# var-nan/SGUFP_Solver

Measured on AMD Instinct MI355X. Metric: B&B-node relaxations/sec + achieved HBM GB/s, 1k-arc 256-scenario synthetic, higher is better.
Workload: dtype f64

## Files before the change

include/sgufp_hip.h:

```cpp
#ifndef SGUFP_HIP_H
#define SGUFP_HIP_H

#include <stdint.h>

#ifdef __cplusplus
extern "C" {
#endif

typedef struct sgufp_ctx sgufp_ctx;

#define SGUFP_OK 0
#define SGUFP_ERR_ARG (-1)
#define SGUFP_ERR_NETWORK (-2)
#define SGUFP_ERR_HIP (-3)
#define SGUFP_ERR_CAPACITY (-4)
#define SGUFP_ERR_STATE (-5)
#define SGUFP_ERR_KEY (-6)

#define SGUFP_SUCCESS 0
#define SGUFP_PRUNED_BY_FEASIBILITY_CUT 1
#define SGUFP_PRUNED_BY_OPTIMALITY_CUT 2
#define SGUFP_NEEDS_SUBPROBLEM 3
#define SGUFP_PRUNED_BY_BOUND 4
#define SGUFP_NODE_ERR_RECORD 16
// ... 33 lines not shown
int sgufp_batch_upload(sgufp_ctx *ctx, int n, const uint16_t *global_layer, const double *lb, const double *ub,
                       const int64_t *states_off, const int16_t *states, const int64_t *sol_off,
                       const int16_t *sol);
int sgufp_batch_relax(sgufp_ctx *ctx, double optimal_lb);
int sgufp_batch_sync(sgufp_ctx *ctx);
int sgufp_batch_results(sgufp_ctx *ctx, int32_t *status, uint8_t *exact, double *lb, double *ub,
                        int32_t *n_children);
int sgufp_batch_children_size(sgufp_ctx *ctx, int64_t *n_children, int64_t *n_states, int64_t *n_sol);
int sgufp_batch_children(sgufp_ctx *ctx, int64_t *child_off, uint16_t *global_layer, double *lb, double *ub,
                         int64_t *states_off, int16_t *states, int64_t *sol_off, int16_t *sol);
int sgufp_batch_paths(sgufp_ctx *ctx, int64_t *path_off, int16_t *paths);
int sgufp_batch_stats(sgufp_ctx *ctx, int64_t *dd_nodes, int64_t *dd_arcs, int32_t *dd_layers, int32_t *sweeps);
int sgufp_batch_refine(sgufp_ctx *ctx, int n, const int32_t *node_idx, const uint8_t *is_feasibility,
                       const int32_t *cut_index, double optimal_lb);

int sgufp_dd_build(sgufp_ctx *ctx);
int sgufp_dd_apply(sgufp_ctx *ctx, int node, int is_feasibility, double rhs, int64_t nnz, const uint64_t *keys,
                   const double *vals, double optimal, double *value);
int sgufp_dd_solution(sgufp_ctx *ctx, int node, int16_t *path, int32_t *len);
int sgufp_dd_cutset(sgufp_ctx *ctx, int node, double ub, int64_t *n_children);

int sgufp_batch_debug(sgufp_ctx *ctx, int64_t *ticks, int32_t *redo);
int sgufp_batch_phases(sgufp_ctx *ctx, int64_t *phase);
int sgufp_batch_refold_stats(sgufp_ctx *ctx, uint32_t *stats);

#define SGUFP_ROUTE_IN_ORDER 0
#define SGUFP_ROUTE_EXACT_PHASE 1
#define SGUFP_ROUTE_NX_PHASE 2
#define SGUFP_ROUTE_NX_FALLBACK 3
int sgufp_batch_routes(sgufp_ctx *ctx, int32_t *route);

int sgufp_subproblem(sgufp_ctx *ctx, int n, const int64_t *path_off, const int16_t *paths, int32_t *type,
                     double *rhs, double *rows, double *obj_mean);
int sgufp_subproblem_detail(sgufp_ctx *ctx, int32_t *status, double *objective, double *dual_objective);
int sgufp_subproblem_warm(sgufp_ctx *ctx, int n, const int64_t *path_off, const int16_t *paths, const int32_t *warm_src,
                          const int32_t *warm_dst, int32_t *type, double *rhs, double *rows, double *obj_mean);
int sgufp_subproblem_stats(sgufp_ctx *ctx, int32_t *augmentations, int32_t *passes);
int sgufp_subproblem_flows(sgufp_ctx *ctx, int n, const int64_t *path_off, const int16_t *paths, int32_t *status,
                           double *objective, double *flow_reward, int16_t *flows, double *mean_flow);
int sgufp_slot_keys(const sgufp_ctx *ctx, uint64_t *keys);
int sgufp_cuts_append_rows(sgufp_ctx *ctx, int is_feasibility, int n_cuts, const double *rhs, const double *rows);

typedef struct {
    int64_t popped;
    int64_t relaxed;
    int64_t pruned_bound;
// ... 74 lines not shown
```

sgufp_solver_amd/csrc/capi.cpp:

```cpp
#include <cstdio>

#include "ctx.hpp"
#include <algorithm>
#include <cstdlib>


namespace {

int64_t node_bound(const Network &net, int64_t *tail = nullptr) {
    const int L = net.L;
    auto set_size = [&](int sid) { return sid >= 0 ? (int)net.sets[sid].size() : 1; };
    int start = std::max(0, L - 5);
    std::vector<int64_t> h(kMaxStates + 2, 0);
    int c0 = set_size(net.layer_universe[start]);
    h[c0] = (L > 5) ? kRelaxedMaxWidth - 1 : 1;
    int64_t total = (int64_t)(kRelaxedMaxWidth - 1) * (start + 1);
    int64_t tail_nodes = 0;
    for (int l = start; l < L; l++) {
        if (net.layer_update[l] >= 0) {
            int64_t w = 0;
            for (auto x : h) w += x;
            std::fill(h.begin(), h.end(), 0);
            h[set_size(net.layer_update[l])] = w;
        }
// ... 97 lines not shown
    if (relax_lds_bytes(sc.Tcap, sc.Lcap, cb, sc.us) > 160 * 1024) { err = "too many layers for the LDS layer table"; return false; }
    sc.tmir_cap = cb > 1 ? (int)(sc.Ncap + sc.Acap) : 0;
    sc.tail_cap = (int)tail;
    sc.cb_max = cb;
    const size_t B = (size_t)max_batch;
    if (!alloc(sc.ntopo, B * sc.Ncap, "scratch") || !alloc(sc.nflag, B * sc.Ncap, "scratch") ||
        !alloc(sc.nmask, B * sc.Ncap, "scratch") || !alloc(sc.outcnt, B * sc.Ncap, "scratch") ||
        !alloc(sc.s2, B * sc.Ncap, "scratch") || !alloc(sc.tw, B * sc.Ncap, "scratch") ||
        !alloc(sc.atopo, B * sc.Acap, "scratch") || !alloc(sc.aflag, B * sc.Acap, "scratch") ||
        !alloc(sc.lay, B * sc.Tcap * 5, "scratch") || !alloc(sc.rslot, B * sc.Lcap, "scratch") ||
        !alloc(sc.meta, B * 8, "scratch") || !alloc(sc.ubv, B, "scratch") ||
        !alloc(sc.sm1, B * sc.Tcap, "scratch") || !alloc(sc.xm1, B * sc.Tcap, "scratch") ||
        !alloc(sc.v1, B * sc.Tcap, "scratch"))
        return false;
    if (cb > 1 && (!alloc(sc.s2b, B * sc.tail_cap * cb, "scratch") || !alloc(sc.sm, B * sc.Tcap * cb, "scratch") ||
                   !alloc(sc.xm, B * sc.Tcap * cb, "scratch") || !alloc(sc.tmir, B * (size_t)sc.tmir_cap, "scratch")))
        return false;
    if (const char *e = getenv("SGUFP_REFOLD_STATS"))
        if (atoi(e) != 0 && cb > 1 && !alloc(sc.rstat, B * kRefoldStats, "scratch")) return false;
    if (!alloc(out.status, B, "out") || !alloc(out.exact, B, "out") || !alloc(out.lb, B, "out") ||
        !alloc(out.ub, B, "out") || !alloc(out.nchild, B, "out") || !alloc(out.sol_need, B, "out") ||
        !alloc(out.dd_nodes, B, "out") || !alloc(out.dd_arcs, B, "out") || !alloc(out.dd_layers, B, "out") ||
        !alloc(out.sweeps, B, "out") || !alloc(out.path, B * sc.Lcap, "out") || !alloc(out.path_len, B, "out") ||
        !alloc(out.ticks, B, "out") || !alloc(out.redo, B, "out") || !alloc(out.phase, B * 8, "out"))
        return false;
    if (!alloc(d_gl, B, "batch") || !alloc(d_sollen, B, "batch") || !alloc(d_lb, B, "batch") ||
        !alloc(d_ub, B, "batch") || !alloc(d_mask, B, "batch") || !alloc(d_valid, B, "batch") ||
        !alloc(d_soloff, B, "batch") || !alloc(d_coff, B + 1, "batch") || !alloc(d_soff, B + 1, "batch") ||
        !alloc(d_rslots, B, "batch") || !alloc(d_rcuts, B, "batch") || !alloc(d_rfeas, B, "batch"))
        return false;
    sol_cap = B * (size_t)std::max(1, L);
    if (!alloc(d_sol, sol_cap, "batch")) return false;
    if (!alloc(d_bidx, B, "bnb") || !alloc(d_boff, B + 1, "bnb") || !alloc(d_bsol, B + 1, "bnb") ||
        !alloc(d_bpaths, B * (size_t)sc.Lcap, "bnb"))
        return false;
    if (!grow_rows(64)) return false;
    cur = staged();
    return sync();
}

bool sgufp_ctx::grow_rows(int need) {
    if (need <= row_cap) return true;
    int cap = std::max(need, row_cap * 2);
    const size_t stride = (size_t)net.n_slots + 1;
    const size_t tstride = (size_t)std::max(net.L, 1) * ustride;
    double *rows = nullptr, *rhs = nullptr, *coefT = nullptr;
    if (!alloc(rows, (size_t)cap * stride, "cut rows") || !alloc(rhs, (size_t)cap, "cut rhs") ||
// ... 1138 lines not shown
    std::vector<int32_t> rows(n);
    for (int k = 0; k < n; k++) {
        const auto &v = is_feasibility[k] ? ctx->f_rows : ctx->o_rows;
        if (node_idx[k] < 0 || node_idx[k] >= ctx->n || cut_index[k] < 0 || cut_index[k] >= (int)v.size())
            return SGUFP_ERR_ARG;
        rows[k] = v[cut_index[k]];
    }
    if (!ctx->upload(ctx->d_rslots, node_idx, n) || !ctx->upload(ctx->d_rcuts, rows.data(), n) ||
        !ctx->upload(ctx->d_rfeas, is_feasibility, n))
        return SGUFP_ERR_HIP;
    if (!ctx->hip_ok(launch_refine(ctx->nd, ctx->sc, ctx->batch(), ctx->pool(), ctx->out, ctx->d_rslots, ctx->d_rcuts,
                                   ctx->d_rfeas, n, optimal_lb, ctx->ex, ctx->stream),
                     "k_refine"))
        return SGUFP_ERR_HIP;
    return ctx->sync() ? SGUFP_OK : SGUFP_ERR_HIP;
}

int sgufp_batch_phases(sgufp_ctx *ctx, int64_t *phase) {
    if (!ctx || !ctx->relaxed || !phase) return ctx ? SGUFP_ERR_STATE : SGUFP_ERR_ARG;
    if (!relax_has_phases()) {
        std::fill(phase, phase + (size_t)ctx->n * 8, (int64_t)0);
        return SGUFP_OK;
    }
    std::vector<uint64_t> t((size_t)ctx->n * 8);
    if (!ctx->download(t.data(), ctx->out.phase, t.size()) || !ctx->sync()) return SGUFP_ERR_HIP;
    for (size_t k = 0; k < t.size(); k++) phase[k] = (int64_t)t[k];
    return SGUFP_OK;
}

int sgufp_batch_refold_stats(sgufp_ctx *ctx, uint32_t *stats) {
    if (!ctx || !stats) return SGUFP_ERR_ARG;
    if (!ctx->relaxed || !ctx->sc.rstat) return SGUFP_ERR_STATE;
    if (!ctx->download(stats, ctx->sc.rstat, (size_t)ctx->n * kRefoldStats) || !ctx->sync()) return SGUFP_ERR_HIP;
    return SGUFP_OK;
}

int sgufp_batch_debug(sgufp_ctx *ctx, int64_t *ticks, int32_t *redo) {
    if (!ctx || !ctx->relaxed) return ctx ? SGUFP_ERR_STATE : SGUFP_ERR_ARG;
    const int n = ctx->n;
    std::vector<uint64_t> t(n);
    std::vector<uint32_t> r(n);
    if (!ctx->download(t.data(), ctx->out.ticks, n) || !ctx->download(r.data(), ctx->out.redo, n) || !ctx->sync())
        return SGUFP_ERR_HIP;
    const bool stamped = relax_has_phases();
    for (int k = 0; k < n; k++) {
        if (ticks) ticks[k] = stamped ? (int64_t)t[k] : 0;
        if (redo) redo[k] = (int32_t)r[k];
    }
    return SGUFP_OK;
// ... 168 lines not shown
```

sgufp_solver_amd/csrc/dd_device.hpp:

```cpp
#pragma once

#include <cstdint>

#if defined(__HIP_DEVICE_COMPILE__) && !defined(SGUFP_HOST_ONLY)
#define SGUFP_GBL __attribute__((address_space(1)))
#else
#define SGUFP_GBL
#endif

namespace sgufp {

constexpr int kWave = 64;
constexpr int kMaxU = 32;
constexpr int kLdsWidth = 512;
constexpr int kBoundBlocks = 1024;

enum NodeStatus : int32_t {
    kSuccess = 0,
    kPrunedFeasibility = 1,
    kPrunedOptimality = 2,
    kNeedsSubproblem = 3,
    kPrunedBound = 4,
    kErrRecord = 16,
    kErrCapacity = 17,
// ... 95 lines not shown
    int ustride;
    const int32_t SGUFP_GBL *o_rank;
    int nscreen;
};

struct BatchOut {
    int32_t SGUFP_GBL *status;
    uint8_t SGUFP_GBL *exact;
    double SGUFP_GBL *lb;
    double SGUFP_GBL *ub;
    uint32_t SGUFP_GBL *nchild;
    uint32_t SGUFP_GBL *sol_need;
    uint32_t SGUFP_GBL *dd_nodes;
    uint32_t SGUFP_GBL *dd_arcs;
    uint32_t SGUFP_GBL *dd_layers;
    uint32_t SGUFP_GBL *sweeps;
    int16_t SGUFP_GBL *path;
    uint16_t SGUFP_GBL *path_len;
    uint64_t SGUFP_GBL *ticks;
    uint64_t SGUFP_GBL *phase;
    uint32_t SGUFP_GBL *redo;
};

struct ChildOut {
    const uint64_t SGUFP_GBL *child_off;
    const uint64_t SGUFP_GBL *sol_base;
    uint16_t SGUFP_GBL *gl;
    double SGUFP_GBL *lb;
    double SGUFP_GBL *ub;
    uint32_t SGUFP_GBL *mask;
    int64_t SGUFP_GBL *sol_off;
    uint16_t SGUFP_GBL *sol_len;
    int16_t SGUFP_GBL *sol;
};

constexpr int32_t kExactPending = 5;
#ifndef SGUFP_EXACT_MAXT
#define SGUFP_EXACT_MAXT 8
#endif
#ifndef SGUFP_EXACT_ENTRIES
#define SGUFP_EXACT_ENTRIES 40
#endif
#ifndef SGUFP_LEAVES_PER_WAVE
#define SGUFP_LEAVES_PER_WAVE 16
#endif
constexpr int kExactMaxT = SGUFP_EXACT_MAXT;
// ... 58 lines not shown
```

sgufp_solver_amd/csrc/dd_kernels.hip:

```cpp
#include <hip/hip_runtime.h>

#include <climits>
#include <cstdint>
#include <type_traits>

#include "dd_device.hpp"
#include "wave.hpp"

namespace sgufp {

#define DMIN (-__DBL_MAX__)
#define DMAX (__DBL_MAX__)

constexpr uint32_t kCollapseWidth = 120;


struct VP {
    double v;
    int p;
};
__device__ __forceinline__ VP vp_pick(VP a, VP b) {
    const bool take_b = (a.p == INT_MIN) | ((b.p != INT_MIN) & ((b.v > a.v) | (!(a.v > b.v) & (b.p > a.p))));
    VP r;
    r.v = take_b ? b.v : a.v;
// ... 695 lines not shown
    }
    for (uint32_t a = lane(); a < d.Amir; a += kWave) {
        uint32_t t = d.atopo[a];
        const bool al = (d.aflag[a] & kAlive) != 0;
        d.tmir[d.Nn + a] = (uint16_t)((al ? (t & kMirParent) : kNarrowMax) | (((t >> kRankShift) & 31u) << kMirRankShift) |
                                      (al ? kMirAlive : 0));
    }
    wave_mem_sync();
}

__device__ __forceinline__ void batch_coef_direct(const NetDev &net, const DD &d, BatchView &bv, const Pool &pool, int k,
                                         int nb) {
    const int us = pool.ustride, ls = d.g + k - 1;
    const size_t ltab = (size_t)net.L * us;
    for (int idx = lane(); idx < nb * us; idx += kWave) {
        int cc = idx / us, r = idx - cc * us;
        bv.coef[idx] = pool.coefT[(size_t)bv.ids[cc] * ltab + (size_t)ls * us + r];
    }
    wave_lds_sync();
}

template <int CB>
__device__ __forceinline__ void sweep_narrow(const NetDev &net, DD &d, BatchView &bv, const Pool &pool, int nb,
                                             double rv, int kS, int kend = INT_MAX) {
    constexpr int G = kWave / CB;
    constexpr int PC = kStageEntries / kWave, PT = kTopoEntries / kWave;
    const int c = lane() % CB, grp = lane() / CB;
    const bool cv = c < nb;
    const int us = pool.ustride;
    const int per_layer = nb * us;
    const size_t ltab = (size_t)net.L * us;
    if (lane() < CB && cv) {
        bv.vb[c] = rv;
        if (c == nb - 1) d.s2[0] = rv;
    }
    if (lane() < 2 * CB)
        bv.vb[(size_t)(lane() / CB) * kLdsBatchWidth * CB + kNarrowMax * CB + (lane() % CB)] = __builtin_nan("");
    if (d.ng == 0) return;
    double pf[PC] = {};
    uint32_t pt[PT] = {};
    uint32_t m_noff = 0, m_aoff = 0, m_pk = 0;
    uint64_t mmask = 0;
    int c_lo[PC];
    uint32_t c_off[PC];
    auto commit = [&](int slot, int gw) {
        LDS double *ring = bv.cring + (size_t)slot * kStageEntries;
        LDS uint16_t *tr = bv.tring + (size_t)slot * kTopoEntries;
// ... 31 lines not shown
        c_lo[jj] = lo | ((r == 0 && lo < 31 ? lo : 31) << 8);
        c_off[jj] = (uint32_t)(bv.ids[cc < nb ? cc : 0] * (int)ltab + r);
    }
    auto issue = [&](int k0g, int k1g, int lw0) {
        const uint32_t n0 = rl(m_noff, k0g - lw0), nN = rl(m_noff, k1g - lw0) - n0;
        const uint32_t a0 = rl(m_aoff, k0g - lw0), nA = rl(m_aoff, k1g - lw0) - a0;
#pragma unroll
        for (int jj = 0; jj < PC; jj++) {
            const int k = min(k0g + (c_lo[jj] & 255), k1g - 1);
            pf[jj] = pool.coefT[(size_t)c_off[jj] + (size_t)(uint32_t)((d.g + k - 1) * us)];
        }
#pragma unroll
        for (int jj = 0; jj < PT; jj++) {
            const uint32_t e = (uint32_t)(lane() + jj * kWave);
            const uint32_t idx = e < nN ? n0 + e : (e < nN + nA ? d.Nn + a0 + (e - nN) : 0u);
            pt[jj] = d.tmir[idx];
        }
    };

    auto fold_run = [&](auto Dc, int ka, int slot_, int k0_, int kw_, uint32_t gn0_) {
        constexpr int D = decltype(Dc)::value;
        const int kb = ka + D - 1;
        const LDS uint16_t *tr = bv.tring + (size_t)slot_ * kTopoEntries;
        const LDS double *ring_c = bv.cring + (size_t)slot_ * kStageEntries + c * us;
        const LDS double *pb = bv.vb + (size_t)((ka - 1) & 1) * kLdsBatchWidth * CB;
        LDS double *ob = bv.vb + (size_t)(kb & 1) * kLdsBatchWidth * CB;
        const int l0 = ka - k0_, lw = ka - kw_;
        uint32_t ebase[D], nofs[D];
        bool w1s[D], wrs[D];
        bool outs = false;
#pragma unroll
        for (int s = 0; s < D; s++) {
            nofs[s] = rl(m_noff, lw + s);
            ebase[s] = nofs[s] - gn0_;
            w1s[s] = (rl(m_pk, lw + s) >> 31) != 0;
            wrs[s] = ((rl(m_pk, lw + s) >> 30) & 1u) != 0;
            outs |= w1s[s] | wrs[s];
        }
        const uint32_t nlast = rl(m_pk, lw + D - 1) & 255u;
        const bool wlane = c == nb - 1;
        auto items = [&](auto Uc, uint32_t base) {
            constexpr int U = decltype(Uc)::value;
            uint32_t cur[U], wl[U][D];
#pragma unroll
            for (int u = 0; u < U; u++) {
                const uint32_t i = base + (uint32_t)(u * G + grp);
                cur[u] = min(i, nlast - 1u);
            }
#pragma unroll
            for (int s = D - 1; s >= 0; s--) {
                uint32_t w[U];
#pragma unroll
                for (int u = 0; u < U; u++) w[u] = (uint32_t)tr[ebase[s] + cur[u]];
                sched_fence();
#pragma unroll
                for (int u = 0; u < U; u++) {
                    wl[u][s] = w[u] | (cur[u] << 16);
                    cur[u] = mir_parent(w[u]);
                }
            }
            double x[U], cf[U][D];
#pragma unroll
            for (int u = 0; u < U; u++) {
                x[u] = pb[cur[u] * CB + c];
#pragma unroll
                for (int s = 0; s < D; s++)
                    cf[u][s] = ring_c[(size_t)(l0 + s) * per_layer + mir_rank(wl[u][s])];
            }
            sched_fence();
#pragma unroll
            for (int u = 0; u < U; u++) {
                double xv = x[u], xs[D];
#pragma unroll
                for (int s = 0; s < D; s++) {
                    const bool in = (wl[u][s] & kMirIn) != 0;
                    xs[s] = xv = in ? xv + cf[u][s] : DMIN;
                }
                ob[(wl[u][D - 1] >> 16) * CB + c] = xv;
                if (outs && (wl[u][D - 1] & kMirAlive) != 0 && cv) {
#pragma unroll
                    for (int s = 0; s < D; s++) {
                        if (w1s[s]) {
                            const uint32_t w = wl[u][s];
                            const bool in = (w & kMirIn) != 0, reg = (w & (31u << kMirRankShift)) != 0;
                            const double xp = s ? xs[s ? s - 1 : 0] : x[u];
                            bv.sm[(size_t)(ka + s) * CB + c] = xs[s];
                            bv.xm[(size_t)(ka + s) * CB + c] = !in ? DMAX : (reg ? xs[s] : xp + 0.0);
                        }
                    }
                    if (wlane) {
#pragma unroll
                        for (int s = 0; s < D; s++)
                            if (wrs[s]) d.s2[nofs[s] + (wl[u][s] >> 16)] = xs[s];
                    }
                }
            }
        };
        const uint32_t per = (nlast + G - 1) / G;
        if (per <= 1) items(std::integral_constant<int, 1>{}, 0u);
        else
            for (uint32_t base = 0; base < nlast; base += 2 * G) items(std::integral_constant<int, 2>{}, base);
    };

    int j = 0, slot = 0;
    int k0 = uni((int)d.gstart[0]), k1 = uni((int)d.gstart[1]);
    int kw = k0;
    load_meta(kw);
    issue(k0, k1, kw);
    commit(0, 0);
    if (d.ng > 1) issue(k1, uni((int)d.gstart[2]), kw);
    uint32_t gn0 = rl(m_noff, 0), gnN = rl(m_noff, k1 - kw) - gn0, ga0 = rl(m_aoff, 0);
    wave_lds_sync();
    const int ke = min(d.kg, kend);
    for (int k = 1; k < ke;) {
        if (k == k1) {
            j++;
            slot ^= 1;
            commit(slot, k1 - kw);
            k0 = k1;
            k1 = uni((int)d.gstart[j + 1]);
            const int k2 = j + 1 < d.ng ? uni((int)d.gstart[j + 2]) : k1;
            if (k2 - kw >= kWave) {
                kw = k0;
                load_meta(kw);
            }
            if (j + 1 < d.ng) issue(k1, k2, kw);
            gn0 = rl(m_noff, k0 - kw);
            gnN = rl(m_noff, k1 - kw) - gn0;
            ga0 = rl(m_aoff, k0 - kw);
            wave_lds_sync();
        }
        const int l = k - k0, lm = k - kw;
        const LDS double *coefk = bv.cring + (size_t)slot * kStageEntries + (size_t)l * per_layer;
        const LDS uint16_t *tr = bv.tring + (size_t)slot * kTopoEntries;
        const uint32_t pk = rl(m_pk, lm);
        const uint32_t noff = rl(m_noff, lm), acnt = (pk >> 8) & 0xFFFu;
        const LDS double *pbuf = bv.vb + (size_t)((k - 1) & 1) * kLdsBatchWidth * CB;
        LDS double *cbuf = bv.vb + (size_t)(k & 1) * kLdsBatchWidth * CB;
        const bool w1 = (pk >> 31) != 0;
        if (acnt) {
            const bool wr = ((pk >> 30) & 1u) != 0;
            const uint32_t aoff = rl(m_aoff, lm);
            const uint32_t ebase = gnN + (aoff - ga0);
            auto word = [&](uint32_t e) -> uint32_t { return (uint32_t)tr[e]; };
            auto dispatch = [&](uint32_t count, auto &&step) {
                uint32_t base = 0;
                for (; count - base > (uint32_t)G * 8; base += G * 8)
                    step(std::integral_constant<int, 8>{}, std::false_type{}, base);
                const uint32_t per = (count - base + G - 1) / G;
                if (per <= 1) step(std::integral_constant<int, 1>{}, std::true_type{}, base);
                else if (per <= 2) step(std::integral_constant<int, 2>{}, std::true_type{}, base);
                else if (per <= 4) step(std::integral_constant<int, 4>{}, std::true_type{}, base);
                else step(std::integral_constant<int, 8>{}, std::true_type{}, base);
// ... 46 lines not shown
                        const uint32_t pp = wd & kMirParent, rr = (wd >> kMirRankShift) & 31u;
                        const bool alive = ok & ((wd & kMirAlive) != 0);
                        const double px = pbuf[(alive ? pp : 0u) * CB + c];
                        const double cf = coefk[(alive ? c * us + rr : 0u)];
                        const bool reg = rr != 0;
                        VP e;
                        e.v = reg ? px + cf : px;
                        e.p = alive ? (reg ? prio_new((int)a) : prio_old((int)a)) : INT_MIN;
                        best = vp_pick(best, e);
                    }
                });
                best = wave_vp<CB>(best);
            }
            if (grp == 0 && cv) {
                double v = (best.p == INT_MIN) ? DMIN : smax(best.v, DMIN);
                cbuf[c] = v;
                if (wr && c == nb - 1) d.s2[noff] = v;
                if (w1) {
                    bv.sm[(size_t)k * CB + c] = v;
                    bv.xm[(size_t)k * CB + c] = any ? xmin : DMAX;
                }
            }
            wave_lds_sync();
            k++;
            continue;
        }
        int kb = min(min(k1, ke) - 1, k + kMaxRun - 1);
        {
            const int span = kb - k + 1;
            const uint64_t b = (mmask >> lm) & ((1ull << span) - 1ull);
            if (b) kb = k + (int)(__ffsll((unsigned long long)b) - 1) - 1;
            if (((kb - k) & 1) != 0) kb--;
        }
        switch (kb - k) {
            case 0: fold_run(std::integral_constant<int, 1>{}, k, slot, k0, kw, gn0); break;
            case 2: fold_run(std::integral_constant<int, 3>{}, k, slot, k0, kw, gn0); break;
            default: fold_run(std::integral_constant<int, 5>{}, k, slot, k0, kw, gn0); break;
        }
        wave_lds_sync();
        k = kb + 1;
    }
}

template <int CB>
__device__ __forceinline__ double batch_value(const DD &d, const BatchView &bv, int k, uint32_t p, int c) {
    if (k >= d.kg) return bv.s2b[(size_t)(uni(d.noff[k]) + p - bv.gbase) * CB + c];
    return bv.vb[(size_t)(k & 1) * kLdsBatchWidth * CB + p * CB + c];
}

template <int CB, bool PV_LDS>
struct ParentVals {
    const LDS double *lds;
    const GBL double *gbl;
    __device__ __forceinline__ void load(uint32_t p, double (&x)[CB]) const {
#pragma unroll
        for (int c = 0; c < CB; c++) x[c] = PV_LDS ? lds[p * CB + c] : gbl[(size_t)p * CB + c];
    }
};
template <int CB, bool PV_LDS>
__device__ __forceinline__ ParentVals<CB, PV_LDS> parent_vals(const DD &d, const BatchView &bv, int k) {
    ParentVals<CB, PV_LDS> pv;
    pv.lds = bv.vb + (size_t)(k & 1) * kLdsBatchWidth * CB;
// ... 517 lines not shown
        sched_fence();
#pragma unroll
        for (int j = 0; j < kFoldBatch; j++)
            if (ok[j]) v = v + x[j];
    }
    return v;
}

__device__ __forceinline__ double root_fold_seq(const Pool &pool, const DD &d, int s0, int total) {
    const int s = min(s0 + lane(), total - 1);
    const int id = seq_id(pool, s);
    return root_fold(pool.rows + (size_t)id * pool.stride, pool.rhs[id], d);
}

struct LoopState {
    int status;
    double ub;
    int last_cut;
    uint32_t applied;
    uint32_t redo;
#ifdef SGUFP_PHASES
    uint64_t ph[8];
    uint64_t t;
    __device__ __forceinline__ void stamp(int k) {
        uint64_t now = wall_clock64();
        ph[k] += now - t;
        t = now;
    }
#else
    __device__ __forceinline__ void stamp(int) {}
#endif
};

__device__ __forceinline__ bool nx_refuse(const ExactIO &ex, int why) {
    if (lane() == 0) atomicAdd(&ex.ctr[9], 1ull << (10 * why));
    return false;
}

__device__ bool nx_compile(const DD &d, const Scratch &sc, const ExactIO &ex, int slot, int &k0_out, int first) {
    const int T = d.T;
    if (T < 3 || d.us > kNxRanks + 1 || !d.stream) return nx_refuse(ex, 0);
    int k0 = 0;
    for (int base = 0; base <= T - 2; base += kWave) {
        const int k = base + lane();
        const uint64_t b = __ballot(k <= T - 2 && d.nalive[k] == 1u);
        if (b) k0 = base + 63 - __clzll((long long)b);
// ... 379 lines not shown
        if (!feas && !screened) {
            screened = true;
            const bool pruned = screen_opt<CB>(net, d, bv, pool, incumbent, st);
            st.stamp(6);
            if (pruned) { st.status = kPrunedOptimality; return; }
        }
        if (!feas && efast) { st.status = kExactPending; return; }
        if (!feas && nx && s >= pool.nf + nx->nx_skip) {
            if (nx_compile(d, sc, *nx, slot, *nx_k0, s - pool.nf)) { st.status = kNxPending; return; }
            nx = nullptr;
        }
        const int nb = min(CB, (feas ? pool.nf : total) - s);
        if (lane() < nb) bv.ids[lane()] = seq_id(pool, s + lane());
        for (int k = lane(); k < d.T; k += kWave) bv.w1[k] = ((d.nalive[k]) == 1) ? 1 : 0;
        int kS = d.T;
        for (int base = 3; base < d.T; base += kWave) {
            int k = base + lane();
            uint64_t b = __ballot(k < d.T && (d.nalive[k]) == 1);
            if (b) { kS = base + (int)(__ffsll((unsigned long long)b) - 1) + 1; break; }
        }
        const double rv = root_fold_seq(pool, d, s, total);
        wave_lds_sync();
        st.stamp(4);
        sweep_narrow<CB>(net, d, bv, pool, nb, rv, kS);
        st.stamp(1);
        if (d.kg == 0 && lane() < nb) bv.s2b[lane()] = rv;
        for (int k = max(d.kg, 1); k < last; k++) sweep_tail_layer<CB>(net, d, bv, pool, k, nb, kS);
        st.stamp(2);
        int next = s + nb;
        if (feas) {
            batch_coef_direct(net, d, bv, pool, last, nb);
            uint32_t rm[CB];
            double mstate[CB];
            f_leaf_scan<CB>(d, bv, pool, nb, kS, rm, mstate);
            st.stamp(3);
            bool removed = false;
            for (int c = 0; c < nb; c++) {
                const int seq = s + c;
                const int id = uni(bv.ids[c]);
                st.last_cut = id;
                st.applied++;
                double maxState = DMIN;
#pragma unroll
                for (int cc = 0; cc < CB; cc++) maxState = (cc == c) ? mstate[cc] : maxState;
                uint32_t rmc = 0;
#pragma unroll
                for (int cc = 0; cc < CB; cc++) rmc = (cc == c) ? rm[cc] : rmc;
// ... 73 lines not shown
                                                double incumbent, ExactIO ex) {
    extern __shared__ __attribute__((aligned(16))) uint8_t smem_raw[];
    LDS uint8_t *smem = (LDS uint8_t *)smem_raw;
    if ((int)blockIdx.x >= in.n) return;
    const int slot = in.perm ? in.perm[blockIdx.x] : (int)blockIdx.x;
    if (ex.redo && out.status[slot] != kNxFallback) return;
    if (sc.rstat && lane() < kRefoldStats) sc.rstat[(size_t)slot * kRefoldStats + lane()] = 0;
#ifdef SGUFP_PHASES
    const uint64_t t_start = wall_clock64();
#endif
    DD d;
    dd_bind(d, smem, sc, slot, CB);
    d.stream = 0;
    d.ng = 0;
    d.kg = 0;
    d.Nn = 0;
    d.Amir = 0;
    d.g = uni((int)in.gl[slot]);
    d.len = uni((int)in.sol_len[slot]);
    const GBL int16_t *rsol = in.sol + in.sol_off[slot];
    d.aligned = (d.len == d.g) ? 1 : 0;
    int cut_layer = 0;
#ifdef SGUFP_PHASES
    LoopState st{kSuccess, in.ub[slot], -1, 0, 0, {0, 0, 0, 0, 0, 0, 0, 0}, t_start};
#else
    LoopState st{kSuccess, in.ub[slot], -1, 0, 0};
#endif
    double lb = DMIN;
    uint32_t nchild = 0, n_nodes = 0, n_arcs = 0, n_merged = 0;
    bool efast = false;
    int nx_k0 = -1;
    d.T = 1; d.exact = 1;

    if (!in.valid[slot] || d.len > d.g || d.g > net.L || d.len > sc.Lcap) {
        st.status = kErrRecord;
        goto done;
    }
    if (in.bound_prune && in.ub[slot] <= incumbent) {
        st.status = kPrunedBound;
        goto done;
    }
    for (int t = lane(); t < d.len; t += kWave) {
        int dec = rsol[t];
        int s = -1;
        if (dec != -1) {
            s = net.n_slots;
            if (dec >= 0 && dec < net.m) {
// ... 83 lines not shown
done:
    if (st.status == kPrunedFeasibility || st.status == kPrunedOptimality || st.status >= kErrRecord) {
        lb = DMIN;
        st.ub = DMIN;
    }
    if (lane() == 0) {
        out.status[slot] = st.status;
        out.exact[slot] = (uint8_t)d.exact;
        out.lb[slot] = lb;
        out.ub[slot] = st.ub;
        out.nchild[slot] = nchild;
        out.sol_need[slot] = nchild * (uint32_t)(d.len + cut_layer);
        out.dd_nodes[slot] = n_nodes;
        out.dd_arcs[slot] = n_arcs;
        out.dd_layers[slot] = (uint32_t)d.T + 1;
        out.sweeps[slot] = st.applied;
        out.redo[slot] = st.redo | (d.stream ? 0x80000000u : 0u) | ((d.Nn + d.Amir) << 8);
    }
    store_meta_layers(d, sc, slot, st.last_cut, st.status, cut_layer, st.ub);
    st.stamp(7);
#ifdef SGUFP_PHASES
    if (lane() == 0) {
        out.ticks[slot] = wall_clock64() - t_start;
        for (int k = 0; k < 8; k++) out.phase[(size_t)slot * 8 + k] = st.ph[k];
    }
#endif
}

__global__ void __launch_bounds__(kWave) k_emit_children(NetDev net, Scratch sc, BatchIn in, Pool pool,
                                                         BatchOut out, ChildOut co) {
    extern __shared__ __attribute__((aligned(16))) uint8_t smem_raw[];
    LDS uint8_t *smem = (LDS uint8_t *)smem_raw;
    const int slot = blockIdx.x;
    if (slot >= in.n) return;
    if (out.status[slot] != kSuccess || out.nchild[slot] == 0) return;
    DD d;
    dd_bind(d, smem, sc, slot);
    load_meta_layers(d, sc, slot);
    const GBL int32_t *meta = sc.meta + (size_t)slot * 8;
    const int last_cut = uni(meta[5]);
    const int k = uni(meta[7]);
    const double ub = sc.ubv[slot];
    const GBL double *row = last_cut >= 0 ? pool.rows + (size_t)last_cut * pool.stride : nullptr;
    const GBL int16_t *rsol = in.sol + in.sol_off[slot];
    const int gl = d.g + k;
    const int stride = d.len + k;
    const bool changed = net.changed[gl] != 0;
// ... 537 lines not shown
```

sgufp_solver_amd/engine.py:

```python
from __future__ import annotations

import ctypes as C
import os
from typing import List, Optional, Sequence, Tuple

import numpy as np

from .pools import DOUBLE_MIN, NodeRecord, PoolCut, RelaxResult

HERE = os.path.dirname(os.path.abspath(__file__))
LIB_PATH = os.environ.get("SGUFP_LIB_PATH") or os.path.join(HERE, "lib", "libsgufp_hip.so")

SUCCESS, PRUNED_F, PRUNED_O, NEEDS_SUBPROBLEM, PRUNED_BOUND = 0, 1, 2, 3, 4
ROUTE_IN_ORDER, ROUTE_EXACT_PHASE, ROUTE_NX_PHASE, ROUTE_NX_FALLBACK = 0, 1, 2, 3
ERR_RECORD, ERR_CAPACITY, ERR_CUTSET = 16, 17, 18

EXPORTS = [
    "sgufp_create_from_file", "sgufp_create", "sgufp_destroy", "sgufp_get_network_info",
    "sgufp_processing_order", "sgufp_last_error", "sgufp_stream", "sgufp_cuts_append",
    "sgufp_cuts_clear", "sgufp_cuts_count", "sgufp_batch_upload", "sgufp_batch_relax",
    "sgufp_batch_sync", "sgufp_batch_results", "sgufp_batch_children_size", "sgufp_batch_children",
    "sgufp_batch_paths", "sgufp_batch_stats", "sgufp_batch_refine", "sgufp_set_timing",
    "sgufp_last_timing", "sgufp_probe_network", "sgufp_batch_debug",
    "sgufp_batch_phases", "sgufp_batch_refold_stats", "sgufp_subproblem", "sgufp_subproblem_detail", "sgufp_slot_keys",
    "sgufp_cuts_append_rows", "sgufp_frontier_clear", "sgufp_frontier_size", "sgufp_frontier_push",
    "sgufp_frontier_take_size", "sgufp_frontier_take", "sgufp_bnb_step", "sgufp_cuts_rows",
    "sgufp_restricted_relax", "sgufp_restricted_results", "sgufp_restricted_paths", "sgufp_restricted_cutset_size",
    "sgufp_restricted_cutset", "sgufp_bnb_set_limits", "sgufp_comm_unique_id", "sgufp_comm_init",
    "sgufp_comm_info", "sgufp_comm_destroy", "sgufp_incumbent_allreduce", "sgufp_cuts_exchange",
    "sgufp_frontier_sizes", "sgufp_frontier_balance", "sgufp_bnb_set_trace", "sgufp_bnb_trace",
    "sgufp_frontier_peek_size", "sgufp_frontier_peek", "sgufp_balance_plan", "sgufp_comm_allgather_i64",
    "sgufp_dd_build", "sgufp_dd_apply", "sgufp_dd_solution", "sgufp_dd_cutset",
    "sgufp_loopback_create", "sgufp_loopback_destroy", "sgufp_comm_init_loopback",
    "sgufp_subproblem_warm", "sgufp_subproblem_stats",
    "sgufp_subproblem_flows", "sgufp_bnb_incumbent", "sgufp_incumbent_set", "sgufp_incumbent_sync", "sgufp_frontier_bound",
]


class BnbStats(C.Structure):
    _fields_ = [(f, C.c_int64) for f in (
        "popped", "relaxed", "pruned_bound", "pruned_feasibility", "pruned_optimality", "exact", "exact_closed",
        "subproblems", "new_feasibility_cuts", "new_optimality_cuts", "children", "pushed", "frontier",
        "dd_nodes", "dd_arcs", "sweeps")] + [("refine_iters", C.c_int32), ("improved", C.c_int32),
                                             ("ms_relax", C.c_double), ("deferred", C.c_int64),
                                             ("resumed", C.c_int64)]

    def as_dict(self):
# ... 47 lines not shown
    lib.sgufp_get_network_info.argtypes = [P, C.POINTER(NetworkInfo)]
    lib.sgufp_processing_order.argtypes = [P, P, P]
    lib.sgufp_last_error.restype = C.c_char_p
    lib.sgufp_last_error.argtypes = [P]
    lib.sgufp_stream.restype = P
    lib.sgufp_stream.argtypes = [P]
    lib.sgufp_cuts_append.argtypes = [P, C.c_int, C.c_int, P, P, P, P]
    lib.sgufp_cuts_clear.argtypes = [P]
    lib.sgufp_cuts_count.argtypes = [P, C.c_int]
    lib.sgufp_batch_upload.argtypes = [P, C.c_int, P, P, P, P, P, P, P]
    lib.sgufp_batch_relax.argtypes = [P, C.c_double]
    lib.sgufp_batch_sync.argtypes = [P]
    lib.sgufp_batch_results.argtypes = [P, P, P, P, P, P]
    lib.sgufp_batch_children_size.argtypes = [P, P, P, P]
    lib.sgufp_batch_children.argtypes = [P, P, P, P, P, P, P, P, P]
    lib.sgufp_batch_paths.argtypes = [P, P, P]
    lib.sgufp_batch_stats.argtypes = [P, P, P, P, P]
    lib.sgufp_batch_refine.argtypes = [P, C.c_int, P, P, P, C.c_double]
    lib.sgufp_set_timing.argtypes = [P, C.c_int]
    lib.sgufp_last_timing.argtypes = [P, P, P]
    lib.sgufp_probe_network.argtypes = [C.c_char_p, P, P, C.c_int32, P, P]
    lib.sgufp_batch_debug.argtypes = [P, P, P]
    lib.sgufp_batch_phases.argtypes = [P, P]
    if hasattr(lib, "sgufp_batch_refold_stats"):
        lib.sgufp_batch_refold_stats.argtypes = [P, P]
    lib.sgufp_batch_routes.argtypes = [P, P]
    lib.sgufp_subproblem.argtypes = [P, C.c_int, P, P, P, P, P, P]
    lib.sgufp_subproblem_detail.argtypes = [P, P, P, P]
    lib.sgufp_slot_keys.argtypes = [P, P]
    lib.sgufp_cuts_append_rows.argtypes = [P, C.c_int, C.c_int, P, P]
    lib.sgufp_frontier_clear.argtypes = [P]
    lib.sgufp_frontier_size.argtypes = [P, P, P]
    lib.sgufp_frontier_push.argtypes = [P, C.c_int, P, P, P, P, P, P, P]
    lib.sgufp_frontier_take_size.argtypes = [P, C.c_int, C.c_int, P, P]
    lib.sgufp_frontier_take.argtypes = [P, C.c_int, C.c_int, P, P, P, P, P, P, P]
    lib.sgufp_bnb_step.argtypes = [P, C.c_int, P, P]
    lib.sgufp_balance_plan.argtypes = [C.c_int, P, P, P, P, P]
    lib.sgufp_comm_allgather_i64.argtypes = [P, P, C.c_int, P]
    lib.sgufp_frontier_peek_size.argtypes = [P, C.c_int64, C.c_int, P, P]
    lib.sgufp_frontier_peek.argtypes = [P, C.c_int64, C.c_int, P, P, P, P, P, P, P]
    lib.sgufp_bnb_set_limits.argtypes = [P, C.c_int, C.c_double]
    lib.sgufp_bnb_set_trace.argtypes = [P, C.c_int]
    lib.sgufp_bnb_trace.argtypes = [P, C.c_int, P, P, P, P, P, P, P, P]
    lib.sgufp_comm_unique_id.argtypes = [P, C.c_int]
    lib.sgufp_comm_init.argtypes = [P, C.c_int, C.c_int, P]
    lib.sgufp_comm_info.argtypes = [P, P, P]
# ... 248 lines not shown
        child_off = np.zeros(n + 1, dtype=np.int64)
        gl = np.zeros(k, dtype=np.uint16)
        lb = np.zeros(k, dtype=np.float64)
        ub = np.zeros(k, dtype=np.float64)
        soff = np.zeros(k + 1, dtype=np.int64)
        states = np.zeros(max(ns.value, 1), dtype=np.int16)
        poff = np.zeros(k + 1, dtype=np.int64)
        sol = np.zeros(max(nsol.value, 1), dtype=np.int16)
        self._check(self.lib.sgufp_batch_children(self.ctx, _ptr(child_off), _ptr(gl), _ptr(lb), _ptr(ub), _ptr(soff),
                                                  _ptr(states), _ptr(poff), _ptr(sol)))
        return child_off, gl, lb, ub, soff, states, poff, sol

    def debug(self):
        t = np.zeros(self.n, dtype=np.int64)
        r = np.zeros(self.n, dtype=np.int32)
        self._check(self.lib.sgufp_batch_debug(self.ctx, _ptr(t), _ptr(r)))
        return t, r

    def phases(self):
        t = np.zeros((self.n, 8), dtype=np.int64)
        self._check(self.lib.sgufp_batch_phases(self.ctx, _ptr(t)))
        return t

    def refold_stats(self):
        t = np.zeros((self.n, 16), dtype=np.uint32)
        self._check(self.lib.sgufp_batch_refold_stats(self.ctx, _ptr(t)))
        return t

    def children_batch(self) -> BatchArrays:
        child_off, gl, lb, ub, soff, states, poff, sol = self.children_arrays()
        return batch_from_arrays(gl, lb, ub, soff, states[:soff[-1]], poff, sol[:poff[-1]])

    def paths(self):
        n = self.n
        off = np.zeros(n + 1, dtype=np.int64)
        self._check(self.lib.sgufp_batch_paths(self.ctx, _ptr(off), None))
        buf = np.zeros(max(int(off[-1]), 1), dtype=np.int16)
        self._check(self.lib.sgufp_batch_paths(self.ctx, _ptr(off), _ptr(buf)))
        return off, buf

    def refine(self, node_idx: Sequence[int], is_feas: Sequence[int], cut_index: Sequence[int], incumbent: float):
        ni = np.asarray(node_idx, dtype=np.int32)
        fe = np.asarray(is_feas, dtype=np.uint8)
        ci = np.asarray(cut_index, dtype=np.int32)
        self._check(self.lib.sgufp_batch_refine(self.ctx, len(ni), _ptr(ni), _ptr(fe), _ptr(ci), C.c_double(incumbent)))

# ... 297 lines not shown
```

Before: 350,600.

## Restructure narrow-sweep fold to per-node lanes with vectorized column loads

Changes the narrow sweep's fold_run so each lane processes a whole DD node across all CB scenario columns, rather than spreading node-by-column pairs across lanes. Prior values are loaded and outputs stored as 2-wide double vectors from LDS. The wr-only case now writes the last column directly instead of recomputing intermediates. It also adds per-phase timing slots for the narrow sweep (under the SGUFP_PHASES build flag) and a C/Python API to read them. This may reduce LDS access overhead and index arithmetic, but it raises register pressure and can leave lanes idle when there are few nodes.

Result: faster. 372,400 (median of 6 runs) (+6.2%).

```diff
diff --git a/include/sgufp_hip.h b/include/sgufp_hip.h
--- a/include/sgufp_hip.h
+++ b/include/sgufp_hip.h
@@ -79,6 +79,7 @@
 
 int sgufp_batch_debug(sgufp_ctx *ctx, int64_t *ticks, int32_t *redo);
 int sgufp_batch_phases(sgufp_ctx *ctx, int64_t *phase);
+int sgufp_batch_narrow_split(sgufp_ctx *ctx, int64_t *split);
 int sgufp_batch_refold_stats(sgufp_ctx *ctx, uint32_t *stats);
 
 #define SGUFP_ROUTE_IN_ORDER 0
diff --git a/sgufp_solver_amd/csrc/capi.cpp b/sgufp_solver_amd/csrc/capi.cpp
--- a/sgufp_solver_amd/csrc/capi.cpp
+++ b/sgufp_solver_amd/csrc/capi.cpp
@@ -143,7 +143,7 @@
         !alloc(out.ub, B, "out") || !alloc(out.nchild, B, "out") || !alloc(out.sol_need, B, "out") ||
         !alloc(out.dd_nodes, B, "out") || !alloc(out.dd_arcs, B, "out") || !alloc(out.dd_layers, B, "out") ||
         !alloc(out.sweeps, B, "out") || !alloc(out.path, B * sc.Lcap, "out") || !alloc(out.path_len, B, "out") ||
-        !alloc(out.ticks, B, "out") || !alloc(out.redo, B, "out") || !alloc(out.phase, B * 8, "out"))
+        !alloc(out.ticks, B, "out") || !alloc(out.redo, B, "out") || !alloc(out.phase, B * kPhaseSlots, "out"))
         return false;
     if (!alloc(d_gl, B, "batch") || !alloc(d_sollen, B, "batch") || !alloc(d_lb, B, "batch") ||
         !alloc(d_ub, B, "batch") || !alloc(d_mask, B, "batch") || !alloc(d_valid, B, "batch") ||
@@ -1328,9 +1328,23 @@
         std::fill(phase, phase + (size_t)ctx->n * 8, (int64_t)0);
         return SGUFP_OK;
     }
-    std::vector<uint64_t> t((size_t)ctx->n * 8);
+    std::vector<uint64_t> t((size_t)ctx->n * kPhaseSlots);
     if (!ctx->download(t.data(), ctx->out.phase, t.size()) || !ctx->sync()) return SGUFP_ERR_HIP;
-    for (size_t k = 0; k < t.size(); k++) phase[k] = (int64_t)t[k];
+    for (size_t i = 0; i < (size_t)ctx->n; i++)
+        for (int k = 0; k < 8; k++) phase[i * 8 + k] = (int64_t)t[i * kPhaseSlots + k];
+    return SGUFP_OK;
+}
+
+int sgufp_batch_narrow_split(sgufp_ctx *ctx, int64_t *split) {
+    if (!ctx || !ctx->relaxed || !split) return ctx ? SGUFP_ERR_STATE : SGUFP_ERR_ARG;
+    if (!relax_has_phases()) {
+        std::fill(split, split + (size_t)ctx->n * 3, (int64_t)0);
+        return SGUFP_OK;
+    }
+    std::vector<uint64_t> t((size_t)ctx->n * kPhaseSlots);
+    if (!ctx->download(t.data(), ctx->out.phase, t.size()) || !ctx->sync()) return SGUFP_ERR_HIP;
+    for (size_t i = 0; i < (size_t)ctx->n; i++)
+        for (int k = 0; k < 3; k++) split[i * 3 + k] = (int64_t)t[i * kPhaseSlots + 8 + k];
     return SGUFP_OK;
 }
 
diff --git a/sgufp_solver_amd/csrc/dd_device.hpp b/sgufp_solver_amd/csrc/dd_device.hpp
--- a/sgufp_solver_amd/csrc/dd_device.hpp
+++ b/sgufp_solver_amd/csrc/dd_device.hpp
@@ -141,6 +141,8 @@
     uint32_t SGUFP_GBL *redo;
 };
 
+constexpr int kPhaseSlots = 11;
+
 struct ChildOut {
     const uint64_t SGUFP_GBL *child_off;
     const uint64_t SGUFP_GBL *sol_base;
diff --git a/sgufp_solver_amd/csrc/dd_kernels.hip b/sgufp_solver_amd/csrc/dd_kernels.hip
--- a/sgufp_solver_amd/csrc/dd_kernels.hip
+++ b/sgufp_solver_amd/csrc/dd_kernels.hip
@@ -741,7 +741,19 @@
 
 template <int CB>
 __device__ __forceinline__ void sweep_narrow(const NetDev &net, DD &d, BatchView &bv, const Pool &pool, int nb,
-                                             double rv, int kS, int kend = INT_MAX) {
+                                             double rv, int kS, int kend = INT_MAX, uint64_t *nclk = nullptr) {
+#ifdef SGUFP_PHASES
+    uint64_t nt = wall_clock64();
+    auto nstamp = [&](int k) {
+        if (nclk) {
+            const uint64_t now = wall_clock64();
+            nclk[k] += now - nt;
+            nt = now;
+        }
+    };
+#else
+    auto nstamp = [](int) {};
+#endif
     constexpr int G = kWave / CB;
     constexpr int PC = kStageEntries / kWave, PT = kTopoEntries / kWave;
     const int c = lane() % CB, grp = lane() / CB;
@@ -819,13 +831,14 @@
         constexpr int D = decltype(Dc)::value;
         const int kb = ka + D - 1;
         const LDS uint16_t *tr = bv.tring + (size_t)slot_ * kTopoEntries;
-        const LDS double *ring_c = bv.cring + (size_t)slot_ * kStageEntries + c * us;
+        const LDS double *ring = bv.cring + (size_t)slot_ * kStageEntries;
         const LDS double *pb = bv.vb + (size_t)((ka - 1) & 1) * kLdsBatchWidth * CB;
         LDS double *ob = bv.vb + (size_t)(kb & 1) * kLdsBatchWidth * CB;
         const int l0 = ka - k0_, lw = ka - kw_;
         uint32_t ebase[D], nofs[D];
         bool w1s[D], wrs[D];
         bool outs = false;
+        bool inner = false;
 #pragma unroll
         for (int s = 0; s < D; s++) {
             nofs[s] = rl(m_noff, lw + s);
@@ -833,17 +846,16 @@
             w1s[s] = (rl(m_pk, lw + s) >> 31) != 0;
             wrs[s] = ((rl(m_pk, lw + s) >> 30) & 1u) != 0;
             outs |= w1s[s] | wrs[s];
+            inner |= w1s[s] | (wrs[s] & (s < D - 1));
         }
         const uint32_t nlast = rl(m_pk, lw + D - 1) & 255u;
-        const bool wlane = c == nb - 1;
-        auto items = [&](auto Uc, uint32_t base) {
+        auto nodes = [&](auto Uc, uint32_t base) {
             constexpr int U = decltype(Uc)::value;
+            constexpr int CC = CB < 4 ? CB : 4, V = CC >= 2 ? 2 : 1;
+            typedef double dv __attribute__((ext_vector_type(V)));
             uint32_t cur[U], wl[U][D];
 #pragma unroll
-            for (int u = 0; u < U; u++) {
-                const uint32_t i = base + (uint32_t)(u * G + grp);
-                cur[u] = min(i, nlast - 1u);
-            }
+            for (int u = 0; u < U; u++) cur[u] = min(base + (uint32_t)(u * kWave + lane()), nlast - 1u);
 #pragma unroll
             for (int s = D - 1; s >= 0; s--) {
                 uint32_t w[U];
@@ -856,47 +868,86 @@
                     cur[u] = mir_parent(w[u]);
                 }
             }
-            double x[U], cf[U][D];
-#pragma unroll
-            for (int u = 0; u < U; u++) {
-                x[u] = pb[cur[u] * CB + c];
-#pragma unroll
-                for (int s = 0; s < D; s++)
-                    cf[u][s] = ring_c[(size_t)(l0 + s) * per_layer + mir_rank(wl[u][s])];
-            }
-            sched_fence();
-#pragma unroll
-            for (int u = 0; u < U; u++) {
-                double xv = x[u], xs[D];
-#pragma unroll
-                for (int s = 0; s < D; s++) {
-                    const bool in = (wl[u][s] & kMirIn) != 0;
-                    xs[s] = xv = in ? xv + cf[u][s] : DMIN;
+#pragma unroll
+            for (int c0 = 0; c0 < CB; c0 += CC) {
+                dv x[U][CC / V];
+                double cf[U][D][CC];
+#pragma unroll
+                for (int u = 0; u < U; u++) {
+#pragma unroll
+                    for (int q = 0; q < CC / V; q++) x[u][q] = *(const LDS dv *)(pb + cur[u] * CB + c0 + q * V);
+#pragma unroll
+                    for (int s = 0; s < D; s++) {
+                        const LDS double *rc = ring + (size_t)(l0 + s) * per_layer + mir_rank(wl[u][s]);
+#pragma unroll
+                        for (int cc = 0; cc < CC; cc++) cf[u][s][cc] = rc[(c0 + cc) * us];
+                    }
                 }
-                ob[(wl[u][D - 1] >> 16) * CB + c] = xv;
-                if (outs && (wl[u][D - 1] & kMirAlive) != 0 && cv) {
-#pragma unroll
-                    for (int s = 0; s < D; s++) {
-                        if (w1s[s]) {
-                            const uint32_t w = wl[u][s];
-                            const bool in = (w & kMirIn) != 0, reg = (w & (31u << kMirRankShift)) != 0;
-                            const double xp = s ? xs[s ? s - 1 : 0] : x[u];
-                            bv.sm[(size_t)(ka + s) * CB + c] = xs[s];
-                            bv.xm[(size_t)(ka + s) * CB + c] = !in ? DMAX : (reg ? xs[s] : xp + 0.0);
+                sched_fence();
+#pragma unroll
+                for (int u = 0; u < U; u++) {
+                    const uint32_t node = wl[u][D - 1] >> 16;
+                    const bool alive = (wl[u][D - 1] & kMirAlive) != 0;
+                    dv xo[CC / V];
+#pragma unroll
+                    for (int cc = 0; cc < CC; cc++) {
+                        double xv = x[u][cc / V][cc % V];
+#pragma unroll
+                        for (int s = 0; s < D; s++) {
+                            const bool in = (wl[u][s] & kMirIn) != 0;
+                            xv = in ? xv + cf[u][s][cc] : DMIN;
+                        }
+                        xo[cc / V][cc % V] = xv;
+                    }
+                    if (outs && alive) {
+                        if (inner) {
+#pragma unroll
+                            for (int cc = 0; cc < CC; cc++) {
+                                const int cq = c0 + cc;
+                                if (cq < nb) {
+                                    const double xp0 = x[u][cc / V][cc % V];
+                                    double xv = xp0, xs[D];
+#pragma unroll
+                                    for (int s = 0; s < D; s++) {
+                                        const bool in = (wl[u][s] & kMirIn) != 0;
+                                        xs[s] = xv = in ? xv + cf[u][s][cc] : DMIN;
+                                    }
+#pragma unroll
+                                    for (int s = 0; s < D; s++) {
+                                        if (w1s[s]) {
+                                            const uint32_t w = wl[u][s];
+                                            const bool in = (w & kMirIn) != 0, reg = (w & (31u << kMirRankShift)) != 0;
+                                            const double xp = s ? xs[s ? s - 1 : 0] : xp0;
+                                            bv.sm[(size_t)(ka + s) * CB + cq] = xs[s];
+                                            bv.xm[(size_t)(ka + s) * CB + cq] = !in ? DMAX : (reg ? xs[s] : xp + 0.0);
+                                        }
+                                    }
+                                    if (cq == nb - 1) {
+#pragma unroll
+                                        for (int s = 0; s < D; s++)
+                                            if (wrs[s]) d.s2[nofs[s] + (wl[u][s] >> 16)] = xs[s];
+                                    }
+                                }
+                            }
+                        } else if (nb - 1 >= c0 && nb - 1 < c0 + CC) {
+                            double v = xo[0][0];
+#pragma unroll
+                            for (int cc = 1; cc < CC; cc++) v = (nb - 1 - c0 == cc) ? xo[cc / V][cc % V] : v;
+                            d.s2[nofs[D - 1] + node] = v;
                         }
                     }
-                    if (wlane) {
-#pragma unroll
-                        for (int s = 0; s < D; s++)
-                            if (wrs[s]) d.s2[nofs[s] + (wl[u][s] >> 16)] = xs[s];
-                    }
+#pragma unroll
+                    for (int q = 0; q < CC / V; q++) *(LDS dv *)(ob + node * CB + c0 + q * V) = xo[q];
                 }
             }
         };
-        const uint32_t per = (nlast + G - 1) / G;
-        if (per <= 1) items(std::integral_constant<int, 1>{}, 0u);
-        else
-            for (uint32_t base = 0; base < nlast; base += 2 * G) items(std::integral_constant<int, 2>{}, base);
+        if constexpr (D == 1) {
+            if (nlast > (uint32_t)kWave) {
+                nodes(std::integral_constant<int, 2>{}, 0u);
+                return;
+            }
+        }
+        for (uint32_t base = 0; base < nlast; base += kWave) nodes(std::integral_constant<int, 1>{}, base);
     };
 
     int j = 0, slot = 0;
@@ -909,6 +960,7 @@
     uint32_t gn0 = rl(m_noff, 0), gnN = rl(m_noff, k1 - kw) - gn0, ga0 = rl(m_aoff, 0);
     wave_lds_sync();
     const int ke = min(d.kg, kend);
+    nstamp(1);
     for (int k = 1; k < ke;) {
         if (k == k1) {
             j++;
@@ -926,6 +978,7 @@
             gnN = rl(m_noff, k1 - kw) - gn0;
             ga0 = rl(m_aoff, k0 - kw);
             wave_lds_sync();
+            nstamp(1);
         }
         const int l = k - k0, lm = k - kw;
         const LDS double *coefk = bv.cring + (size_t)slot * kStageEntries + (size_t)l * per_layer;
@@ -1018,6 +1071,7 @@
                 }
             }
             wave_lds_sync();
+            nstamp(0);
             k++;
             continue;
         }
@@ -1034,6 +1088,7 @@
             default: fold_run(std::integral_constant<int, 5>{}, k, slot, k0, kw, gn0); break;
         }
         wave_lds_sync();
+        nstamp(2);
         k = kb + 1;
     }
 }
@@ -1597,6 +1652,7 @@
 #ifdef SGUFP_PHASES
     uint64_t ph[8];
     uint64_t t;
+    uint64_t ns[3];
     __device__ __forceinline__ void stamp(int k) {
         uint64_t now = wall_clock64();
         ph[k] += now - t;
@@ -2022,7 +2078,11 @@
         const double rv = root_fold_seq(pool, d, s, total);
         wave_lds_sync();
         st.stamp(4);
+#ifdef SGUFP_PHASES
+        sweep_narrow<CB>(net, d, bv, pool, nb, rv, kS, INT_MAX, st.ns);
+#else
         sweep_narrow<CB>(net, d, bv, pool, nb, rv, kS);
+#endif
         st.stamp(1);
         if (d.kg == 0 && lane() < nb) bv.s2b[lane()] = rv;
         for (int k = max(d.kg, 1); k < last; k++) sweep_tail_layer<CB>(net, d, bv, pool, k, nb, kS);
@@ -2142,7 +2202,7 @@
     d.aligned = (d.len == d.g) ? 1 : 0;
     int cut_layer = 0;
 #ifdef SGUFP_PHASES
-    LoopState st{kSuccess, in.ub[slot], -1, 0, 0, {0, 0, 0, 0, 0, 0, 0, 0}, t_start};
+    LoopState st{kSuccess, in.ub[slot], -1, 0, 0, {0, 0, 0, 0, 0, 0, 0, 0}, t_start, {0, 0, 0}};
 #else
     LoopState st{kSuccess, in.ub[slot], -1, 0, 0};
 #endif
@@ -2272,7 +2332,8 @@
 #ifdef SGUFP_PHASES
     if (lane() == 0) {
         out.ticks[slot] = wall_clock64() - t_start;
-        for (int k = 0; k < 8; k++) out.phase[(size_t)slot * 8 + k] = st.ph[k];
+        for (int k = 0; k < 8; k++) out.phase[(size_t)slot * kPhaseSlots + k] = st.ph[k];
+        for (int k = 0; k < 3; k++) out.phase[(size_t)slot * kPhaseSlots + 8 + k] = st.ns[k];
     }
 #endif
 }
diff --git a/sgufp_solver_amd/engine.py b/sgufp_solver_amd/engine.py
--- a/sgufp_solver_amd/engine.py
+++ b/sgufp_solver_amd/engine.py
@@ -22,7 +22,7 @@
     "sgufp_batch_sync", "sgufp_batch_results", "sgufp_batch_children_size", "sgufp_batch_children",
     "sgufp_batch_paths", "sgufp_batch_stats", "sgufp_batch_refine", "sgufp_set_timing",
     "sgufp_last_timing", "sgufp_probe_network", "sgufp_batch_debug",
-    "sgufp_batch_phases", "sgufp_batch_refold_stats", "sgufp_subproblem", "sgufp_subproblem_detail", "sgufp_slot_keys",
+    "sgufp_batch_phases", "sgufp_batch_narrow_split", "sgufp_batch_refold_stats", "sgufp_subproblem", "sgufp_subproblem_detail", "sgufp_slot_keys",
     "sgufp_cuts_append_rows", "sgufp_frontier_clear", "sgufp_frontier_size", "sgufp_frontier_push",
     "sgufp_frontier_take_size", "sgufp_frontier_take", "sgufp_bnb_step", "sgufp_cuts_rows",
     "sgufp_restricted_relax", "sgufp_restricted_results", "sgufp_restricted_paths", "sgufp_restricted_cutset_size",
@@ -116,6 +116,7 @@
     lib.sgufp_probe_network.argtypes = [C.c_char_p, P, P, C.c_int32, P, P]
     lib.sgufp_batch_debug.argtypes = [P, P, P]
     lib.sgufp_batch_phases.argtypes = [P, P]
+    lib.sgufp_batch_narrow_split.argtypes = [P, P]
     if hasattr(lib, "sgufp_batch_refold_stats"):
         lib.sgufp_batch_refold_stats.argtypes = [P, P]
     lib.sgufp_batch_routes.argtypes = [P, P]
@@ -410,6 +411,11 @@
         self._check(self.lib.sgufp_batch_phases(self.ctx, _ptr(t)))
         return t
 
+    def narrow_split(self):
+        t = np.zeros((self.n, 3), dtype=np.int64)
+        self._check(self.lib.sgufp_batch_narrow_split(self.ctx, _ptr(t)))
+        return t
+
     def refold_stats(self):
         t = np.zeros((self.n, 16), dtype=np.uint32)
         self._check(self.lib.sgufp_batch_refold_stats(self.ctx, _ptr(t)))
```
